# tjqansthd/GDN-Pytorch

Measured on AMD Instinct MI355X. Metric: training images/sec at 128x416 batch=20, higher is better.
Workload: dtype f32; 1 GPU; DtoD training step (fwd + losses + bwd + fused Adam), batch 20 per GPU, 128x416, fp32, BASELINE configs[1]; global_batch=20, parallelism=dp1, launch=eager, x3=True

## Files before the change

### gdn-pytorch_amd/csrc/conv_wino.hip

```cpp
#include "common.h"
#include "wino_gemm.h"
#include "up2x.h"
#include "gemm_x3.h"

namespace {

struct WinoGeom {
    int B, H, W, C, N;
    int Ho, Wo;
    int pad_off;
    int reflect;
    int tiles_y, tiles_x, M;
    int cq_shift, nq_shift;
    int x3;
    int flip;
    int T, bins;
};

__global__ __launch_bounds__(256) void wino_input_kernel(const float* __restrict__ x, int ldx, float* __restrict__ V, WinoGeom g,
                                                         const float* __restrict__ in_scale, const float* __restrict__ in_shift,
                                                         int in_relu, int up2x) {
    int t, c;
    if (!wino_decode(g.M, g.cq_shift, t, c)) return;
    const float is = in_scale ? in_scale[c] : 1.f, it = in_scale ? in_shift[c] : 0.f;
// ... 718 lines not shown
    WinoGeom f;
    if (!wino_geom(g, f)) return GDN_ERR_UNSUPPORTED;
    if (!dy || (!dx && !dw) || (dx && !w && !state) || (dw && !state)) return GDN_ERR_BAD_ARG;
    if (bnb_y && (!dx || !bnb_co || !bnb_partial)) return GDN_ERR_BAD_ARG;
    if (bnb_y && f.reflect) return GDN_ERR_UNSUPPORTED;
    if (dx && f.reflect && ((ldx % 4) || (addsrc && (ld_add % 4)))) return GDN_ERR_UNSUPPORTED;
    if (dx_up2x < 0 || dx_up2x > 2 || (dx_up2x && ((g->H & 1) || (g->W & 1)))) return GDN_ERR_BAD_ARG;
    if (dx && dx_up2x && !f.reflect) return GDN_ERR_UNSUPPORTED;
    if (!workspace || workspace_bytes < gdn_winoconv_bwd_workspace_bytes(g)) return GDN_ERR_WORKSPACE;
    hipStream_t st = (hipStream_t)stream;
    char* p = (char*)workspace;
    const size_t Md = f.reflect ? (size_t)f.B * cdiv(f.H + 2, 2) * cdiv(f.W + 2, 2) : (size_t)f.M;
    const size_t vd = al256((size_t)f.bins * Md * f.N * 4);
    float* Vd = (float*)p; p += (vd > m_bytes(f) ? vd : m_bytes(f));
    float* U = (float*)p; p += u_bytes(f);
    float* Eo = (float*)p;
    if (f.T == 4) {
        if (dw) {
            hipLaunchKernelGGL(wino4_dy_kernel, dim3(cdiv(f.M, 4) << f.nq_shift), dim3(256), 0, st, dy, ldy, Vd, f);
            const int ns = tn_splits(f);
            launch_gemm_x3_tn((const float*)Vd, (const float*)state, Eo, f.bins, f.M, f.N, f.C, ns, st);
            hipLaunchKernelGGL(wino4_wgrad_output_kernel, dim3(cdiv(f.N * f.C, 256)), dim3(256), 0, st, (const float*)Eo, dw, f.N, f.C, ns, f.flip ? 1 : 0);
        }
        if (dx) {
            WinoGeom fd = f;
            fd.C = f.N; fd.N = f.C; fd.cq_shift = f.nq_shift; fd.nq_shift = f.cq_shift;
            hipLaunchKernelGGL(wino4_input_kernel, dim3(cdiv(fd.M, 4) << fd.cq_shift), dim3(256), 0, st, dy, ldy, Vd, fd,
                               (const float*)nullptr, (const float*)nullptr, 0, 0);
            const float* Ud = U;
            if (state) Ud = (const float*)((const char*)state + v_bytes(f));
            else hipLaunchKernelGGL(wino4_weights_x3_kernel, dim3(cdiv(f.N * f.C / 8, 256)), dim3(256), 0, st, w, (unsigned char*)U, f.N, f.C, 1 | f.flip,
                                    (unsigned char*)nullptr, 0);
            launch_gemm_x3_nt((const float*)Vd, Ud, Eo, f.bins, fd.M, f.C, f.N, st);
            hipLaunchKernelGGL(wino4_output_kernel, dim3(cdiv(fd.M, 4) << fd.nq_shift), dim3(256), 0, st, (const float*)Eo, dx, ldx,
                               addsrc, ld_add, bnb_y ? bnb_partial : (float*)nullptr, (const float*)nullptr, (const float*)nullptr, 0,
                               fd, f.C, fd.nq_shift, bnb_y, ld_bnb, bnb_co, bnb_relu);
        }
        return gdn_launch_status();
    }
    if (dw) {
        hipLaunchKernelGGL(wino_dy_kernel, dim3(cdiv(f.M, 4) << f.nq_shift), dim3(256), 0, st, dy, ldy, Vd, f);
        const int ns = tn_splits(f);
        if (tn_x3(f)) launch_gemm_x3_tn((const float*)Vd, (const float*)state, Eo, WINO_BINS, f.M, f.N, f.C, ns, st);
        else launch_wino_gemm_tn((const float*)Vd, (const float*)state, Eo, f.M, f.N, f.C, ns, st);
        hipLaunchKernelGGL(wino_wgrad_output_kernel, dim3(cdiv(f.N * f.C, 256)), dim3(256), 0, st, (const float*)Eo, dw, f.N, f.C, ns, f.flip ? 1 : 0);
    }
    if (dx) {
        WinoGeom fd = f;
        fd.C = f.N; fd.N = f.C; fd.cq_shift = f.nq_shift; fd.nq_shift = f.cq_shift; fd.reflect = 0;
        float* out = dx;
        int ld_out = ldx;
        if (f.reflect) {
            fd.Ho = f.H + 2; fd.Wo = f.W + 2; fd.pad_off = 2;
            fd.tiles_y = cdiv(fd.Ho, 2); fd.tiles_x = cdiv(fd.Wo, 2); fd.M = f.B * fd.tiles_y * fd.tiles_x;
            out = Eo + (size_t)WINO_BINS * fd.M * f.C;
            ld_out = f.C;
        }
        hipLaunchKernelGGL(wino_input_kernel, dim3(cdiv(fd.M, 4) << fd.cq_shift), dim3(256), 0, st, dy, ldy, Vd, fd,
                           (const float*)nullptr, (const float*)nullptr, 0, 0);
        const float* Ud = U;
        const bool x3d = f.x3 && gemm_x3_ok(f.M, f.C, f.N);
        if (state) Ud = (const float*)((const char*)state + v_bytes(f));
        else if (x3d) hipLaunchKernelGGL(wino_weights_x3_kernel, dim3(cdiv(f.N * f.C / 8, 256)), dim3(256), 0, st, w, (unsigned char*)U, f.N, f.C, 1 | f.flip,
                                         (unsigned char*)nullptr, 0);
        else hipLaunchKernelGGL(wino_weights_kernel, dim3(cdiv(f.N * f.C, 256)), dim3(256), 0, st, w, U, f.N, f.C, 1 | f.flip, (float*)nullptr);
        if (x3d) launch_gemm_x3_nt((const float*)Vd, Ud, Eo, WINO_BINS, fd.M, f.C, f.N, st);
        else launch_wino_gemm((const float*)Vd, Ud, Eo, fd.M, f.C, f.N, st);
        hipLaunchKernelGGL(wino_output_kernel, dim3(cdiv(fd.M, 4) << fd.nq_shift), dim3(256), 0, st, (const float*)Eo, out, ld_out,
                           f.reflect ? (const float*)nullptr : addsrc, ld_add, bnb_y ? bnb_partial : (float*)nullptr,
                           (const float*)nullptr, (const float*)nullptr, 0, fd, f.C, fd.nq_shift, bnb_y, ld_bnb, bnb_co, bnb_relu);
        if (f.reflect && dx_up2x) {
            const int64_t nb = cdiv64((int64_t)f.B * (f.H / 2) * (f.W / 2) * (f.C / 4), 256);
            hipLaunchKernelGGL(reflect_fold_up2x_kernel, dim3((unsigned)(nb < 65536 * 8 ? nb : 65536 * 8)), dim3(256), 0, st,
                               (const void*)out, (void*)dx, ldx, (const void*)addsrc, ld_add, f.B, f.H, f.W, f.C, 1, dx_up2x - 1, 0);
        } else if (f.reflect) {
            const int64_t nb = cdiv64((int64_t)f.B * f.H * f.W * (f.C / 4), 256);
            hipLaunchKernelGGL(wino_reflect_fold_kernel, dim3((unsigned)(nb < 65536 * 8 ? nb : 65536 * 8)), dim3(256), 0, st,
                               (const float*)out, dx, ldx, addsrc, ld_add, f.B, f.H, f.W, f.C);
        }
    }
    return gdn_launch_status();
}

extern "C" int gdn_winoconv_gemm(const gdn_conv_geom* g, const float* V, const float* U, float* Mo, void* stream) {
    (void)hipGetLastError();
    WinoGeom f;
    if (!wino_geom(g, f)) return GDN_ERR_UNSUPPORTED;
    if (!V || !U || !Mo) return GDN_ERR_BAD_ARG;
    launch_wino_gemm(V, U, Mo, f.B * cdiv(f.H, 2) * cdiv(f.W, 2), f.N, f.C, (hipStream_t)stream);
    return gdn_launch_status();
}
```

### gdn-pytorch_amd/gdn_amd/_lib.py

```python
import ctypes
import os
import pathlib
from ctypes import POINTER, Structure, c_char_p, c_float, c_int32, c_int64, c_size_t, c_uint64, c_void_p

_PKG = pathlib.Path(__file__).resolve().parent
LIB_PATH = pathlib.Path(os.environ.get("GDN_HIP_LIB", _PKG.parent / "lib" / "libgdn_hip.so"))


class GdnError(RuntimeError):
    pass


class ConvGeom(Structure):
    _fields_ = [("B", c_int32), ("H", c_int32), ("W", c_int32), ("Cin", c_int32), ("Cout", c_int32),
                ("k", c_int32), ("stride", c_int32), ("pad", c_int32), ("pad_mode", c_int32),
                ("transposed", c_int32), ("hints", c_int32)]


_PG = POINTER(ConvGeom)
_P = c_void_p
_i32, _i64, _f, _sz = c_int32, c_int64, c_float, c_size_t

_SIGS = {
    "gdn_version": (c_int32, []),
    "gdn_hints_supported": (c_int32, []),
    "gdn_strerror": (c_char_p, [c_int32]),
    "gdn_device_info": (c_int32, [c_char_p, c_int32]),
    "gdn_conv_out_dims": (c_int32, [_PG, POINTER(c_int32), POINTER(c_int32)]),
    "gdn_conv_stats_slots": (_i64, [_PG, _i32]),
    "gdn_conv_fwd_workspace_bytes": (_sz, [_PG, _i32]),
    "gdn_conv_fwd": (c_int32, [_PG, _P, _i32, _P, _i32, _i32, _P, _P, _i32, _P, _i32, _P, _P, _P, _i32, _i32, _P, _sz, _P]),
    "gdn_conv_dgrad_workspace_bytes": (_sz, [_PG, _i32]),
    "gdn_conv_dgrad": (c_int32, [_PG, _P, _i32, _P, _P, _i32, _P, _i32, _P, _i32, _P, _i32, _P, _i32, _P, _sz, _i32, _P]),
    "gdn_conv_dgrad_bnb_slots": (_i64, [_PG, _i32]),
    "gdn_conv_wgrad_workspace_bytes": (_sz, [_PG, _i32]),
    "gdn_conv_wgrad": (c_int32, [_PG, _P, _i32, _i32, _P, _i32, _P, _i32, _i32, _P, _sz, _i32, _P]),
    "gdn_conv_wgrad_bf16_workspace_bytes": (_sz, [_PG, _i32, _i32]),
    "gdn_conv_wgrad_bf16": (c_int32, [_PG, _P, _i32, _i32, _P, _i32, _P, _i32, _i32, _P, _sz, _i32, _P]),
    "gdn_fftconv_fwd_workspace_bytes": (_sz, [_PG]),
    "gdn_fftconv_spectrum_bytes": (_sz, [_PG]),
    "gdn_fftconv_stats_slots": (_i64, [_PG]),
    "gdn_fftconv_fwd": (c_int32, [_PG, _P, _i32, _P, _P, _i32, _P, _i32, _P, _P, _P, _i32, _P, _P, _i32, _i32, _P, _P, _sz, _P]),
    "gdn_fftconv_bwd_workspace_bytes": (_sz, [_PG]),
    "gdn_fftconv_bwd": (c_int32, [_PG, _P, _i32, _P, _P, _P, _i32, _P, _i32, _P, _P, _i32, _P, _P, _i32, _P, _i32, _P, _i32, _P,
                                  _i32, _i32, _P, _sz, _P]),
    "gdn_fftconv_bnb_slots": (_i64, [_PG]),
    "gdn_fftconv_cgemm_workspace_bytes": (_sz, [_PG]),
    "gdn_fftconv_cgemm": (c_int32, [_PG, _i32, _P, _sz, _P]),
    "gdn_fftconv_cgemm_shape": (c_int32, [_PG, _P, _P, _P]),
    "gdn_winoconv_fwd_workspace_bytes": (_sz, [_PG]),
    "gdn_winoconv_state_bytes": (_sz, [_PG]),
    "gdn_winoconv_stats_slots": (_i64, [_PG]),
    "gdn_winoconv_fwd": (c_int32, [_PG, _P, _i32, _P, _P, _i32, _P, _i32, _P, _P, _P, _i32, _P, _P, _i32, _i32, _P, _P, _sz, _P]),
    "gdn_winoconv_bwd_workspace_bytes": (_sz, [_PG]),
    "gdn_winoconv_bnb_slots": (_i64, [_PG]),
    "gdn_winoconv_gemm": (c_int32, [_PG, _P, _P, _P, _P]),
    "gdn_winoconv_bwd": (c_int32, [_PG, _P, _i32, _P, _P, _P, _i32, _P, _i32, _P, _P, _i32, _P, _i32, _P, _i32, _P, _sz, _P]),
    "gdn_wino2conv_fwd_workspace_bytes": (_sz, [_PG]),
    "gdn_wino2conv_state_bytes": (_sz, [_PG]),
    "gdn_wino2conv_stats_slots": (_i64, [_PG]),
    "gdn_wino2conv_fwd": (c_int32, [_PG, _P, _i32, _P, _P, _i32, _P, _i32, _P, _P, _P, _i32, _P, _P, _sz, _P]),
    "gdn_wino2conv_bwd_workspace_bytes": (_sz, [_PG]),
    "gdn_wino2conv_bwd": (c_int32, [_PG, _P, _i32, _P, _P, _i32, _P, _P, _i32, _P, _i32, _P, _P, _sz, _P]),
    "gdn_conv_c1_stats_slots": (_i64, [_i32, _i32, _i32]),
    "gdn_conv_c1_fwd": (c_int32, [_P, _i32, _i32, _i32, _i32, _i32, _i32, _i32, _i32, _i32, _P, _P, _i32, _P, _i32, _P, _P, _P, _i32,
                                  _i32, _P]),
    "gdn_conv_c1_wgrad_workspace_bytes": (_sz, []),
    "gdn_conv_c1_wgrad": (c_int32, [_P, _P, _i32, _i32, _i32, _i32, _i32, _i32, _i32, _i32, _i32, _i32, _P, _P, _sz, _P]),
    "gdn_gemm_x3_packed_bytes": (_sz, [_i32, _i32, _i32]),
    "gdn_gemm_x3_pack": (c_int32, [_P, _P, _i32, _i32, _i32, _P]),
    "gdn_gemm_x3_nt": (c_int32, [_P, _P, _P, _i32, _i32, _i32, _i32, _P]),
    "gdn_gemm_x3_tn": (c_int32, [_P, _P, _P, _i32, _i32, _i32, _i32, _i32, _P]),
    "gdn_gemm_x3_tn_splits": (_i64, [_i32, _i32, _i32, _i32]),
    "gdn_transpose_taps": (c_int32, [_P, _P, _i32, _i32, _i32, _i32, _P]),
    "gdn_cast": (c_int32, [_P, _P, _i64, _i32, _P]),
    "gdn_weight_to_tapmajor": (c_int32, [_P, _P, _i32, _i32, _i32, _i32, _P]),
    "gdn_weight_from_tapmajor": (c_int32, [_P, _P, _i32, _i32, _i32, _i32, _P]),
    "gdn_bn_finalize_train": (c_int32, [_P, _i64, _i32, _i64, _P, _P, _P, _P, _f, _f, _P, _P, _P, _P, _P, _P]),
    "gdn_bn_eval_coeffs": (c_int32, [_P, _P, _P, _P, _f, _i32, _P, _P, _P]),
    "gdn_bn_apply": (c_int32, [_P, _i32, _P, _P, _P, _i32, _P, _i32, _i64, _i32, _i32, _i32, _P]),
    "gdn_bn_bwd_workspace_bytes": (_sz, [_i64, _i32]),
    "gdn_bn_bwd": (c_int32, [_P, _i32, _P, _i32, _P, _P, _P, _P, _P, _P, _i32, _P, _P, _i64, _i32, _i32, _P, _i64, _P, _sz, _i32, _P]),
    "gdn_bn_bwd_coeffs": (c_int32, [_P, _i32, _P, _i32, _P, _P, _P, _P, _P, _P, _P, _i64, _i32, _i32, _P, _i64, _P, _sz, _i32, _P]),
    "gdn_bn_eval_bwd": (c_int32, [_P, _i32, _P, _i32, _P, _P, _P, _i32, _i64, _i32, _i32, _i32, _P]),
    "gdn_bn_apply_up2x": (c_int32, [_P, _P, _P, _P, _P, _P, _i32, _i32, _i32, _i32, _i32, _i32, _i32, _P]),
    "gdn_upsample2x_fwd": (c_int32, [_P, _P, _i32, _i32, _i32, _i32, _i32, _i32, _P]),
    "gdn_upsample2x_bwd": (c_int32, [_P, _P, _i32, _i32, _i32, _i32, _i32, _i32, _P]),
    "gdn_nchw_to_nhwc": (c_int32, [_P, _P, _i32, _i32, _i32, _i32, _i32, _P]),
    "gdn_nhwc_to_nchw": (c_int32, [_P, _P, _i32, _i32, _i32, _i32, _i32, _P]),
    "gdn_add": (c_int32, [_P, _P, _P, _i64, _i32, _P]),
    "gdn_add_pitched": (c_int32, [_P, _i32, _P, _i32, _P, _i32, _i64, _i32, _i32, _P]),
    "gdn_scale_dev": (c_int32, [_P, _P, _P, _i64, _P]),
    "gdn_tanh_bwd": (c_int32, [_P, _P, _P, _i64, _P]),
    "gdn_fill": (c_int32, [_P, _f, _i64, _P]),
    "gdn_loss_workspace_bytes": (_sz, [_i64]),
    "gdn_absdiff_max": (c_int32, [_P, _P, _i64, _P, _P]),
    "gdn_berhu_masked": (c_int32, [_P, _P, _P, _i32, _i32, _i32, _i32, POINTER(c_int32), _P, _P, _P, _P, _sz, _P]),
    "gdn_sobel_l1": (c_int32, [_P, _P, _i32, _i32, _i32, _f, _P, _P, _P, _P, _P, _sz, _P]),
    "gdn_smoothness": (c_int32, [_P, _P, _i32, _i32, _i32, _i32, _P, _P, _P, _P, _P, _P, _sz, _P]),
    "gdn_mse": (c_int32, [_P, _P, _i64, _f, _i32, _P, _P, _sz, _i32, _P]),
    "gdn_kitti_augment_workspace_bytes": (_sz, [_i32]),
    "gdn_kitti_augment": (c_int32, [_P, _i32, _i32, _i32, _i32, _i32, _P, _i32, _P, _P, _sz, _P]),
    "gdn_kitti_augment_resident": (c_int32, [_P, _i32, _P, _i32, _P, _i32, _i32, _i32, _P, _i32, _i32, _P, _P, _P, _P]),
    "gdn_gather_samples": (c_int32, [_P, _i32, _P, _i32, _i64, _i32, _P, _P]),
    "gdn_mse_grad": (c_int32, [_P, _P, _i64, _f, _P, _P, _i32, _P]),
    "gdn_depth_metrics_workspace_bytes": (_sz, [_i32, _i32, _i32]),
    "gdn_depth_metrics": (c_int32, [_P, _P, _P, _i32, _i32, _i32, _i32, _P, _P, _sz, _P]),
    "gdn_depth_metrics_nyu_workspace_bytes": (_sz, [_i32, _i32, _i32]),
    "gdn_depth_metrics_nyu": (c_int32, [_P, _P, _i32, _i32, _i32, _i32, _P, _P, _sz, _P]),
    "gdn_depth_metrics_make3d_workspace_bytes": (_sz, [_i32, _i32, _i32]),
    "gdn_depth_metrics_make3d": (c_int32, [_P, _P, _P, _i32, _i32, _i32, _P, _P, _sz, _P]),
    "gdn_crop_normalize": (c_int32, [_P, _i32, _i32, _i32, _i32, _i32, _i32, _i32, _i32, _i32, _P, _P]),
    "gdn_bytescale_u8": (c_int32, [_P, _i32, _i32, _i32, _i32, _P, _P]),
    "gdn_nyu_augment_workspace_bytes": (_sz, [_i32, _i32, _i32, _i32]),
    "gdn_nyu_augment": (c_int32, [_P, _P, _i32, _i32, _i32, _i32, _P, _i32, _i32, _P, _P, _P, _sz, _P]),
    "gdn_pil_resize_workspace_bytes": (_sz, [_i32, _i32, _i32, _i32]),
    "gdn_pil_resize_bilinear": (c_int32, [_P, _i32, _i32, _i32, _i32, _i32, _i32, _i32, _i32, _i32, _i32, _i32, _i32, _i32,
                                          _P, _P, _sz, _P]),
    "gdn_spline_rotate3_workspace_bytes": (_sz, [_i32, _i32, _i32, _i32]),
    "gdn_spline_rotate3": (c_int32, [_P, _i32, _i32, _i32, _i32, _P, _P, _i32, _P, _P, _sz, _P]),
    "gdn_adam_step": (c_int32, [_P, _P, _P, _P, _i64, _f, _f, _f, _f, _f, _i32, _f, _P]),
    "gdn_adam_step_dev": (c_int32, [_P, _P, _P, _P, _i64, _P, _P, _P]),
    "gdn_clock_probe_arm": (c_int32, [_P, _P]),
    "gdn_clock_probe_watch": (c_int32, [_P, c_uint64, _P]),
    "gdn_clock_probe_stop": (c_int32, [_P, _P]),
}
_STATUS_FUNCS = {n for n, (r, _) in _SIGS.items() if r is c_int32} - {"gdn_version", "gdn_device_info", "gdn_hints_supported"}

EXPORTS = tuple(_SIGS)
ABI_VERSION = 223


class _Lib:
    def __init__(self):
        self._dll = None

    def _load(self):
        if self._dll is not None:
            return self._dll
        if not LIB_PATH.exists():
# ... 38 lines not shown
```

### gdn-pytorch_amd/gdn_amd/ops.py

```python
import ctypes
import math
import os

import numpy as np
import torch

from ._lib import ConvGeom, GdnError, lib

ACT_NONE, ACT_TANH, ACT_RELU = 0, 1, 2
BN_EPS, BN_MOMENTUM = 1e-5, 0.1


def stream():
    return torch.cuda.current_stream().cuda_stream


def _p(t):
    return None if t is None else t.data_ptr()


def _is_bf16(t):
    return 1 if t is not None and t.dtype == torch.bfloat16 else 0


# ... 359 lines not shown
                         device=dy.device) if need_dx else None
        ws = workspace(nb, dy.device, "fft")
        yy, yco, ykk, yrelu = dyb if dyb is not None else (None, None, None, False)

        def call(phases, st):
            lib.gdn_fftconv_bwd(ref, _p(dy), _ld(dy), _p(w_tap), _p(xf), _p(dx),
                                0 if dx is None else _ld(dx), _p(addsrc), 0 if addsrc is None else _ld(addsrc),
                                _p(dw_tap), _p(yy), 0 if yy is None else _ld(yy), _p(yco), _p(ykk), 1 if yrelu else 0,
                                _p(by), 0 if by is None else _ld(by), _p(bco), 1 if brelu else 0, _p(bpart),
                                int(up2x), phases, _p(ws), nb, st)
        if dw_tap is not None and need_dx:
            main = torch.cuda.current_stream(dy.device)
            side = side_stream(dy.device)
            call(1, main.cuda_stream)
            side.wait_stream(main)
            call(2, side.cuda_stream)
            call(4, main.cuda_stream)
            main.wait_stream(side)
        else:
            call(0, stream())
        return dx

    def fft_cgemm_only(self, B, H, W, which, ws=None, train=False, st=None):
        _, ref, _, _ = self.geom(B, H, W, hints=HINT_TRAIN if train else 0)
        nb = int(lib.gdn_fftconv_cgemm_workspace_bytes(ref))
        if nb == 0:
            raise GdnError("fftconv: unsupported layer k=%d stride=%d" % (self.k, self.stride))
        if ws is None:
            ws = torch.empty(nb // 4, dtype=torch.float32, device="cuda").normal_()
        lib.gdn_fftconv_cgemm(ref, int(which), _p(ws), nb, stream() if st is None else st)
        bins, M, npnt = ctypes.c_int32(), ctypes.c_int32(), ctypes.c_int32()
        lib.gdn_fftconv_cgemm_shape(ref, ctypes.byref(bins), ctypes.byref(M), ctypes.byref(npnt))
        return ws, bins.value, M.value, npnt.value

    def wino_ok(self, B, H, W, backward=False):
        _, ref, _, _ = self.geom(B, H, W)
        if backward:
            return int(lib.gdn_winoconv_bwd_workspace_bytes(ref)) > 0
        return int(lib.gdn_winoconv_state_bytes(ref)) > 0

    def wino_fwd(self, x, w_tap, stats=False, addsrc=None, state=False, affine=None, act=ACT_NONE, in_affine=None,
                 in_relu=False, up2x=0):
        _chk(x, "x"); _chk(w_tap, "w")
        B, H, W, C1 = x.shape
        if up2x:
            H, W = 2 * H, 2 * W
        _, ref, Ho, Wo = self.geom(B, H, W)
        nb = int(lib.gdn_winoconv_fwd_workspace_bytes(ref))
        if nb == 0 or C1 != self.cin:
            raise GdnError("winoconv: unsupported layer k=%d stride=%d Cin=%d Cout=%d" % (self.k, self.stride, C1, self.cout))
        y = torch.empty((B, Ho, Wo, self.cout), dtype=torch.float32, device=x.device)
        st = torch.empty((int(lib.gdn_winoconv_stats_slots(ref)), 2, self.cout), dtype=torch.float32,
                         device=x.device) if stats else None
        sv = torch.empty(int(lib.gdn_winoconv_state_bytes(ref)), dtype=torch.uint8, device=x.device) if state else None
        if sv is not None:
            sv._gdn_x3 = _x3
            sv._gdn_f4 = _f4
        ws = workspace(nb, x.device, "fft")
        lib.gdn_winoconv_fwd(ref, _p(x), _ld(x), _p(w_tap), _p(y), _ld(y), _p(addsrc), 0 if addsrc is None else _ld(addsrc),
                             _p(st), _p(affine[0]) if affine else None, _p(affine[1]) if affine else None, int(act),
                             _p(in_affine[0]) if in_affine else None, _p(in_affine[1]) if in_affine else None,
                             1 if in_relu else 0, int(up2x), _p(sv), _p(ws), nb, stream())
        res = (y,) + ((st,) if stats else ()) + ((sv,) if state else ())
        return res if len(res) > 1 else y

    def wino_gemm_only(self, V, U, Mo, B, H, W):
        _, ref, _, _ = self.geom(B, H, W)
        lib.gdn_winoconv_gemm(ref, _p(V), _p(U), _p(Mo), stream())

    def wino_bwd(self, dy, w_tap, in_hw, state=None, dw_tap=None, need_dx=True, addsrc=None, bnb=None, up2x=0):
        _chk(dy, "dy")
        B = dy.shape[0]
        H, W = in_hw
        _, ref, Ho, Wo = self.geom(B, H, W, x3=_state_x3(state), f4=_state_f4(state))
        nb = int(lib.gdn_winoconv_bwd_workspace_bytes(ref))
        if nb == 0:
            raise GdnError("winoconv: unsupported layer k=%d stride=%d" % (self.k, self.stride))
        if tuple(dy.shape[1:]) != (Ho, Wo, self.cout):
            raise GdnError("wino_bwd: dy shape %s does not match layer output" % (tuple(dy.shape),))
        if bnb is not None and not need_dx:
            raise GdnError("wino_bwd: bnb needs the data gradient (need_dx)")
        dx = torch.empty((B, H // 2, W // 2, self.cin) if up2x else (B, H, W, self.cin), dtype=torch.float32,
                         device=dy.device) if need_dx else None
        ws = workspace(nb, dy.device, "fft")
        by, bco, brelu, bpart = bnb if bnb is not None else (None, None, False, None)
        lib.gdn_winoconv_bwd(ref, _p(dy), _ld(dy), _p(w_tap), _p(state), _p(dx), 0 if dx is None else _ld(dx), _p(addsrc),
                             0 if addsrc is None else _ld(addsrc), _p(dw_tap), _p(by), 0 if by is None else _ld(by), _p(bco),
                             1 if brelu else 0, _p(bpart), int(up2x), _p(ws), nb, stream())
        return dx

    def wino2_ok(self, B, H, W):
        _, ref, _, _ = self.geom(B, H, W)
        return int(lib.gdn_wino2conv_fwd_workspace_bytes(ref)) > 0

    def wino2_fwd(self, x, w_tap, stats=False, addsrc=None, state=False, affine=None, act=ACT_NONE):
        _chk(x, "x"); _chk(w_tap, "w")
        B, H, W, C1 = x.shape
        _, ref, Ho, Wo = self.geom(B, H, W)
        nb = int(lib.gdn_wino2conv_fwd_workspace_bytes(ref))
        if nb == 0 or C1 != self.cin:
            raise GdnError("wino2conv: unsupported layer k=%d stride=%d Cin=%d Cout=%d" % (self.k, self.stride, C1, self.cout))
        y = torch.empty((B, Ho, Wo, self.cout), dtype=torch.float32, device=x.device)
        st = torch.empty((int(lib.gdn_wino2conv_stats_slots(ref)), 2, self.cout), dtype=torch.float32,
                         device=x.device) if stats else None
        sv = None
        if state:
            sb = int(lib.gdn_wino2conv_state_bytes(ref))
            sv = torch.empty(sb, dtype=torch.uint8, device=x.device) if sb else x
        ws = workspace(nb, x.device, "fft")
        lib.gdn_wino2conv_fwd(ref, _p(x), _ld(x), _p(w_tap), _p(y), _ld(y), _p(addsrc), 0 if addsrc is None else _ld(addsrc),
                              _p(st), _p(affine[0]) if affine else None, _p(affine[1]) if affine else None, int(act),
                              _p(sv) if (sv is not None and sv is not x) else None, _p(ws), nb, stream())
        res = (y,) + ((st,) if stats else ()) + ((sv,) if state else ())
        return res if len(res) > 1 else y

    def wino2_bwd(self, dy, w_tap, in_hw, state=None, dw_tap=None, need_dx=True, addsrc=None, bnb=None):
        _chk(dy, "dy")
        B = dy.shape[0]
        H, W = in_hw
        _, ref, Ho, Wo = self.geom(B, H, W)
        nb = int(lib.gdn_wino2conv_bwd_workspace_bytes(ref))
        if nb == 0:
            raise GdnError("wino2conv: unsupported layer k=%d stride=%d" % (self.k, self.stride))
        if tuple(dy.shape[1:]) != (Ho, Wo, self.cout):
            raise GdnError("wino2_bwd: dy shape %s does not match layer output" % (tuple(dy.shape),))
        dx = torch.empty((B, H, W, self.cin), dtype=torch.float32, device=dy.device) if need_dx else None
        ws = workspace(nb, dy.device, "fft")
        xin = state if self.transposed else None
        sv = None if self.transposed else state
        lib.gdn_wino2conv_bwd(ref, _p(dy), _ld(dy), _p(w_tap), _p(xin), 0 if xin is None else _ld(xin), _p(sv), _p(dx),
                              0 if dx is None else _ld(dx), _p(addsrc), 0 if addsrc is None else _ld(addsrc), _p(dw_tap),
                              _p(ws), nb, stream())
        return dx

    def wgrad(self, x, dy, dw_tap, ci_off=0, cfg=0):
        _chk(x, "x", bf16_ok=True)
        _chk(dy, "dy", bf16_ok=True)
        _chk(dw_tap, "dw")
        B, H, W, Cx = x.shape
        _, ref, _, _ = self.geom(B, H, W)
        if x.dtype == torch.bfloat16 and dy.dtype == torch.bfloat16:
            nb = int(lib.gdn_conv_wgrad_bf16_workspace_bytes(ref, Cx, cfg))
            if nb == 0:
                raise GdnError("bf16 wgrad: unsupported geometry k=%d stride=%d Cx=%d Cout=%d" % (self.k, self.stride, Cx, self.cout))
            ws = workspace(nb, x.device, "wgrad")
            lib.gdn_conv_wgrad_bf16(ref, _p(x), _ld(x), Cx, _p(dy), _ld(dy), _p(dw_tap), self.cin, ci_off, _p(ws), nb, cfg,
                                    stream())
            return
        nb = int(lib.gdn_conv_wgrad_workspace_bytes(ref, Cx))
        if nb == 0:
            raise GdnError("wgrad: unsupported geometry k=%d stride=%d Cx=%d" % (self.k, self.stride, Cx))
        ws = workspace(nb, x.device, "wgrad")
        lib.gdn_conv_wgrad(ref, _p(x), _ld(x), Cx, _p(dy), _ld(dy), _p(dw_tap), self.cin, ci_off, _p(ws), nb,
                           _mask(x, dy), stream())


def c1_ok(x1, n, k, stride, pad, rgb=False):
    return (x1.dtype == torch.float32 and x1.dim() == 4 and (x1.shape[3] == 1 or (rgb and x1.shape[3] == 3)) and x1.is_contiguous()
            and n == 64 and k == 9 and stride == 1 and pad == 4)


def conv_c1_fwd(x1, w81, reflect=False, flip=False, stats=False, addsrc=None, affine=None, act=ACT_NONE, out_dtype=torch.float32):
    _chk(x1, "x1"); _chk(w81, "w")
    if x1.dtype != torch.float32 or w81.dtype != torch.float32:
        raise GdnError("conv_c1_fwd: the image and the weights are fp32")
    B, H, W, cin = x1.shape
    if cin not in (1, 3) or w81.numel() != 81 * 64 * cin or not w81.is_contiguous() or not x1.is_contiguous():
        raise GdnError("conv_c1_fwd: dense [B,H,W,1|3] image and 81 x 64 x Cin contiguous weights expected")
# ... 520 lines not shown
```

### include/gdn_hip.h

```cpp
#ifndef GDN_HIP_H
#define GDN_HIP_H

#include <stddef.h>
#include <stdint.h>

#ifdef __cplusplus
extern "C" {
#endif

typedef enum {
    GDN_OK = 0,
    GDN_ERR_BAD_ARG = -1,
    GDN_ERR_UNSUPPORTED = -2,
    GDN_ERR_WORKSPACE = -3,
    GDN_ERR_LAUNCH = -4
} gdn_status;

int gdn_version(void);
int gdn_hints_supported(void);
const char* gdn_strerror(int status);
int gdn_device_info(char* name, int name_len);

typedef struct {
    int32_t B, H, W;
    int32_t Cin, Cout;
    int32_t k, stride, pad;
    int32_t pad_mode;
    int32_t transposed;
    int32_t hints;
} gdn_conv_geom;

enum { GDN_HINT_TRAIN = 1, GDN_HINT_NO_X3 = 2, GDN_HINT_NO_WINO_F4 = 4, GDN_HINT_FFT_NP32 = 8, GDN_HINT_FFT_NP40 = 16,
       GDN_HINT_FLIP_TAPS = 32 };
#define GDN_HINT_PLAN_BATCH(n) (((n) & 0xff) << 8)
#define GDN_HINT_PLAN_CUS(n) ((((n) / 8) & 0xff) << 16)

enum { GDN_ACT_NONE = 0, GDN_ACT_TANH = 1, GDN_ACT_RELU = 2 };

enum { GDN_CFG_KC64 = 0x200, GDN_CFG_NO_SPLITK = 0x800, GDN_CFG_BF16 = 0x10000 };

int gdn_conv_out_dims(const gdn_conv_geom* g, int32_t* Ho, int32_t* Wo);

int64_t gdn_conv_stats_slots(const gdn_conv_geom* g, int32_t tile_cfg);

size_t gdn_conv_fwd_workspace_bytes(const gdn_conv_geom* g, int32_t tile_cfg);
int gdn_conv_fwd(const gdn_conv_geom* g,
                 const void* x, int32_t ldx, const void* x2, int32_t ldx2, int32_t C1,
                 const void* w, void* y, int32_t ldy,
                 const void* addsrc, int32_t ld_add,
                 float* stats, const float* ep_scale, const float* ep_shift, int32_t act, int32_t tile_cfg,
                 void* workspace, size_t workspace_bytes, void* stream);

size_t gdn_conv_dgrad_workspace_bytes(const gdn_conv_geom* g, int32_t tile_cfg);
int64_t gdn_conv_dgrad_bnb_slots(const gdn_conv_geom* g, int32_t tile_cfg);
int gdn_conv_dgrad(const gdn_conv_geom* g, const void* dy, int32_t ldy,
                   const void* wt, void* dx, int32_t ldx,
                   const void* addsrc, int32_t ld_add,
                   const void* bnb_y, int32_t ld_bnb, const float* bnb_co, int32_t bnb_relu, float* bnb_partial,
                   int32_t dx_up2x, void* workspace, size_t workspace_bytes, int32_t tile_cfg, void* stream);

size_t gdn_conv_wgrad_workspace_bytes(const gdn_conv_geom* g, int32_t Cx);
int gdn_conv_wgrad(const gdn_conv_geom* g, const void* x, int32_t ldx, int32_t Cx,
                   const void* dy, int32_t ldy,
                   float* dw, int32_t ld_dw, int32_t ci_off,
                   void* workspace, size_t workspace_bytes, int32_t dtypes, void* stream);

size_t gdn_fftconv_fwd_workspace_bytes(const gdn_conv_geom* g);
size_t gdn_fftconv_spectrum_bytes(const gdn_conv_geom* g);
int64_t gdn_fftconv_stats_slots(const gdn_conv_geom* g);
int gdn_fftconv_fwd(const gdn_conv_geom* g, const float* x, int32_t ldx, const float* w,
                    float* y, int32_t ldy, const float* addsrc, int32_t ld_add, float* stats,
                    const float* ep_scale, const float* ep_shift, int32_t act,
                    const float* in_scale, const float* in_shift, int32_t in_relu, int32_t in_up2x,
                    void* xf_out, void* workspace, size_t workspace_bytes, void* stream);
enum { GDN_FFT_BWD_TRANSFORM = 1, GDN_FFT_BWD_DW = 2, GDN_FFT_BWD_DX = 4, GDN_FFT_BWD_ALL = 7 };
size_t gdn_fftconv_bwd_workspace_bytes(const gdn_conv_geom* g);
int gdn_fftconv_bwd(const gdn_conv_geom* g, const float* dy, int32_t ldy, const float* w,
                    const void* xf, float* dx, int32_t ldx, const float* addsrc, int32_t ld_add,
                    float* dw, const float* dyb_y, int32_t ld_dyb, const float* dyb_co,
                    const float* dyb_kk, int32_t dyb_relu,
                    const float* bnb_y, int32_t ld_bnb, const float* bnb_co, int32_t bnb_relu, float* bnb_partial,
                    int32_t dx_up2x, int32_t phases,
                    void* workspace, size_t workspace_bytes, void* stream);
int64_t gdn_fftconv_bnb_slots(const gdn_conv_geom* g);
size_t gdn_fftconv_cgemm_workspace_bytes(const gdn_conv_geom* g);
int gdn_fftconv_cgemm(const gdn_conv_geom* g, int32_t which, void* workspace, size_t workspace_bytes, void* stream);
int gdn_fftconv_cgemm_shape(const gdn_conv_geom* g, int32_t* bins, int32_t* M, int32_t* np);

size_t gdn_winoconv_fwd_workspace_bytes(const gdn_conv_geom* g);
size_t gdn_winoconv_state_bytes(const gdn_conv_geom* g);
int64_t gdn_winoconv_stats_slots(const gdn_conv_geom* g);
int gdn_winoconv_fwd(const gdn_conv_geom* g, const float* x, int32_t ldx, const float* w,
                     float* y, int32_t ldy, const float* addsrc, int32_t ld_add, float* stats,
                     const float* ep_scale, const float* ep_shift, int32_t act,
                     const float* in_scale, const float* in_shift, int32_t in_relu, int32_t in_up2x,
                     void* state_out, void* workspace, size_t workspace_bytes, void* stream);
size_t gdn_winoconv_bwd_workspace_bytes(const gdn_conv_geom* g);
int64_t gdn_winoconv_bnb_slots(const gdn_conv_geom* g);
int gdn_winoconv_gemm(const gdn_conv_geom* g, const float* V, const float* U, float* Mo, void* stream);
int gdn_winoconv_bwd(const gdn_conv_geom* g, const float* dy, int32_t ldy, const float* w,
                     const void* state, float* dx, int32_t ldx, const float* addsrc, int32_t ld_add,
                     float* dw, const float* bnb_y, int32_t ld_bnb, const float* bnb_co, int32_t bnb_relu,
                     float* bnb_partial, int32_t dx_up2x, void* workspace, size_t workspace_bytes, void* stream);

size_t gdn_wino2conv_fwd_workspace_bytes(const gdn_conv_geom* g);
size_t gdn_wino2conv_state_bytes(const gdn_conv_geom* g);
int64_t gdn_wino2conv_stats_slots(const gdn_conv_geom* g);
int gdn_wino2conv_fwd(const gdn_conv_geom* g, const float* x, int32_t ldx, const float* w,
                      float* y, int32_t ldy, const float* addsrc, int32_t ld_add, float* stats,
                      const float* ep_scale, const float* ep_shift, int32_t act,
                      void* state_out, void* workspace, size_t workspace_bytes, void* stream);
size_t gdn_wino2conv_bwd_workspace_bytes(const gdn_conv_geom* g);
int gdn_wino2conv_bwd(const gdn_conv_geom* g, const float* dy, int32_t ldy, const float* w,
                      const float* x, int32_t ldx_in, const void* state,
                      float* dx, int32_t ldx, const float* addsrc, int32_t ld_add, float* dw,
                      void* workspace, size_t workspace_bytes, void* stream);

int64_t gdn_conv_c1_stats_slots(int32_t B, int32_t H, int32_t W);
int gdn_conv_c1_fwd(const float* x1, int32_t Cin, int32_t B, int32_t H, int32_t W, int32_t N, int32_t k, int32_t pad, int32_t reflect,
                    int32_t flip, const float* w, void* y, int32_t ldy, const void* addsrc, int32_t ld_add,
                    float* stats, const float* ep_scale, const float* ep_shift, int32_t act, int32_t dtypes, void* stream);
size_t gdn_conv_c1_wgrad_workspace_bytes(void);
int gdn_conv_c1_wgrad(const float* x1, const void* gw, int32_t ldg, int32_t gw_bf16, int32_t B, int32_t H, int32_t W, int32_t N,
                      int32_t k, int32_t pad, int32_t reflect, int32_t flip, float* dw,
                      void* workspace, size_t workspace_bytes, void* stream);

size_t gdn_gemm_x3_packed_bytes(int32_t bins, int32_t rows, int32_t K);
int gdn_gemm_x3_pack(const float* src, void* dst, int32_t bins, int32_t rows, int32_t K, void* stream);
int gdn_gemm_x3_nt(const float* A, const void* Bp, float* C, int32_t bins, int32_t M, int32_t N, int32_t K, void* stream);
int gdn_gemm_x3_tn(const float* A, const float* B, float* P, int32_t bins, int32_t T, int32_t NI, int32_t NJ, int32_t nsplit,
                   void* stream);
int64_t gdn_gemm_x3_tn_splits(int32_t bins, int32_t T, int32_t NI, int32_t NJ);

size_t gdn_conv_wgrad_bf16_workspace_bytes(const gdn_conv_geom* g, int32_t Cx, int32_t cfg);
int gdn_conv_wgrad_bf16(const gdn_conv_geom* g, const void* x, int32_t ldx, int32_t Cx,
                        const void* dy, int32_t ldy,
                        float* dw, int32_t ld_dw, int32_t ci_off,
                        void* workspace, size_t workspace_bytes, int32_t cfg, void* stream);


int gdn_transpose_taps(const void* w, void* wt, int32_t ntaps, int32_t R, int32_t C, int32_t dtypes, void* stream);
int gdn_cast(const void* src, void* dst, int64_t n, int32_t dtypes, void* stream);
int gdn_weight_to_tapmajor(const float* w_torch, float* w_tap, int32_t Cout, int32_t Cin, int32_t ntaps,
                           int32_t a_is_cout, void* stream);
int gdn_weight_from_tapmajor(const float* w_tap, float* w_torch, int32_t Cout, int32_t Cin, int32_t ntaps,
                             int32_t a_is_cout, void* stream);

int gdn_bn_finalize_train(const float* stats, int64_t slots, int32_t C, int64_t count,
                          const float* gamma, const float* beta,
                          float* running_mean, float* running_var, float momentum, float eps,
                          float* scale, float* shift, float* mean, float* invstd,
                          int64_t* num_batches_tracked, void* stream);
int gdn_bn_eval_coeffs(const float* gamma, const float* beta, const float* running_mean,
                       const float* running_var, float eps, int32_t C,
                       float* scale, float* shift, void* stream);
int gdn_bn_apply(const void* y, int32_t ldy, const float* scale, const float* shift,
                 const void* residual, int32_t ld_res, void* out, int32_t ld_out,
                 int64_t npix, int32_t C, int32_t relu, int32_t dtypes, void* stream);
int gdn_bn_apply_up2x(const void* y, const float* scale, const float* shift, const void* residual, void* low, void* up,
                      int32_t B, int32_t H, int32_t W, int32_t C, int32_t relu, int32_t align_corners, int32_t dtypes,
                      void* stream);
size_t gdn_bn_bwd_workspace_bytes(int64_t npix, int32_t C);
int gdn_bn_bwd(const void* dout, int32_t ld_dout, const void* y, int32_t ldy,
               const float* gamma, const float* scale, const float* shift,
               const float* mean, const float* invstd,
               void* dy, int32_t ld_dy, float* dgamma, float* dbeta,
               int64_t npix, int32_t C, int32_t relu,
               const float* ext_partial, int64_t ext_slots,
               void* workspace, size_t workspace_bytes, int32_t dtypes, void* stream);

int gdn_bn_bwd_coeffs(const void* dout, int32_t ld_dout, const void* y, int32_t ldy,
                      const float* scale, const float* shift, const float* mean, const float* invstd,
                      float* dgamma, float* dbeta, float* kk, int64_t npix, int32_t C, int32_t relu,
                      const float* ext_partial, int64_t ext_slots,
                      void* workspace, size_t workspace_bytes, int32_t dtypes, void* stream);

int gdn_bn_eval_bwd(const void* dout, int32_t ld_dout, const void* y, int32_t ldy,
                    const float* scale, const float* shift, void* dy, int32_t ld_dy,
                    int64_t npix, int32_t C, int32_t relu, int32_t dtypes, void* stream);

int gdn_upsample2x_fwd(const void* x, void* y, int32_t B, int32_t H, int32_t W, int32_t C,
                       int32_t align_corners, int32_t dtypes, void* stream);
int gdn_upsample2x_bwd(const void* dy, void* dx, int32_t B, int32_t H, int32_t W, int32_t C,
                       int32_t align_corners, int32_t dtypes, void* stream);

int gdn_nchw_to_nhwc(const void* x, void* y, int32_t B, int32_t C, int32_t H, int32_t W, int32_t dtypes, void* stream);
// ... 100 lines not shown
```

Measured before the change: 528.5 images/s.

## Overlap Winograd-4 weight-grad and data-grad GEMMs on separate streams

Adds a phased Winograd F(4) backward entry point that splits the input transforms, the weight-gradient GEMM and reduction, and the data-gradient GEMM and output transform into selectable phases. The Python wrapper runs the transforms on the main stream, then the wgrad phase on a side stream while dgrad runs on the main stream, and joins the two afterwards. The aim is to fill GPU idle time by running the two independent backward GEMMs at the same time. In exchange it needs a larger workspace holding both transformed buffers, adds stream synchronisation overhead, and skips the up2x and non-T=4 cases.

```diff
diff --git a/gdn-pytorch_amd/csrc/conv_wino.hip b/gdn-pytorch_amd/csrc/conv_wino.hip
--- a/gdn-pytorch_amd/csrc/conv_wino.hip
+++ b/gdn-pytorch_amd/csrc/conv_wino.hip
@@ -824,6 +824,63 @@
     return gdn_launch_status();
 }
 
+namespace {
+inline size_t pair_vd_bytes(const WinoGeom& f) { return al256((size_t)f.bins * f.M * f.N * 4); }
+inline size_t pair_p_bytes(const WinoGeom& f) { return (size_t)tn_splits_max(f) * al256((size_t)f.bins * f.N * f.C * 4); }
+inline size_t pair_eo_bytes(const WinoGeom& f) { return al256((size_t)f.bins * f.M * f.C * 4); }
+inline bool pair_geom(const gdn_conv_geom* g, WinoGeom& f) { return wino_geom(g, f) && f.T == 4; }
+}
+
+extern "C" size_t gdn_winoconv_bwd_pair_workspace_bytes(const gdn_conv_geom* g) {
+    WinoGeom f;
+    if (!pair_geom(g, f)) return 0;
+    return 2 * pair_vd_bytes(f) + pair_p_bytes(f) + pair_eo_bytes(f);
+}
+
+extern "C" int gdn_winoconv_bwd_pair(const gdn_conv_geom* g, const float* dy, int32_t ldy, const float* w, const void* state,
+                                     float* dx, int32_t ldx, const float* addsrc, int32_t ld_add, float* dw,
+                                     const float* bnb_y, int32_t ld_bnb, const float* bnb_co, int32_t bnb_relu,
+                                     float* bnb_partial, int32_t dx_up2x, int32_t phases, void* workspace, size_t workspace_bytes,
+                                     void* stream) {
+    (void)hipGetLastError();
+    (void)w;
+    WinoGeom f;
+    if (!pair_geom(g, f)) return GDN_ERR_UNSUPPORTED;
+    if (!dy || !dx || !dw || !state) return GDN_ERR_BAD_ARG;
+    if (bnb_y && (!bnb_co || !bnb_partial)) return GDN_ERR_BAD_ARG;
+    if (dx_up2x < 0 || dx_up2x > 2) return GDN_ERR_BAD_ARG;
+    if (dx_up2x) return GDN_ERR_UNSUPPORTED;
+    if (phases < 0 || phases > 7) return GDN_ERR_BAD_ARG;
+    if (!workspace || workspace_bytes < gdn_winoconv_bwd_pair_workspace_bytes(g)) return GDN_ERR_WORKSPACE;
+    if (!phases) phases = 7;
+    hipStream_t st = (hipStream_t)stream;
+    char* p = (char*)workspace;
+    float* Vd = (float*)p; p += pair_vd_bytes(f);
+    float* Dv = (float*)p; p += pair_vd_bytes(f);
+    float* P = (float*)p; p += pair_p_bytes(f);
+    float* Eo = (float*)p;
+    WinoGeom fd = f;
+    fd.C = f.N; fd.N = f.C; fd.cq_shift = f.nq_shift; fd.nq_shift = f.cq_shift;
+    if (phases & 1) {
+        hipLaunchKernelGGL(wino4_input_kernel, dim3(cdiv(fd.M, 4) << fd.cq_shift), dim3(256), 0, st, dy, ldy, Vd, fd,
+                           (const float*)nullptr, (const float*)nullptr, 0, 0);
+        hipLaunchKernelGGL(wino4_dy_kernel, dim3(cdiv(f.M, 4) << f.nq_shift), dim3(256), 0, st, dy, ldy, Dv, f);
+    }
+    if (phases & 2) {
+        const int ns = tn_splits(f);
+        launch_gemm_x3_tn((const float*)Dv, (const float*)state, P, f.bins, f.M, f.N, f.C, ns, st);
+        hipLaunchKernelGGL(wino4_wgrad_output_kernel, dim3(cdiv(f.N * f.C, 256)), dim3(256), 0, st, (const float*)P, dw, f.N, f.C, ns, f.flip ? 1 : 0);
+    }
+    if (phases & 4) {
+        const float* Ud = (const float*)((const char*)state + v_bytes(f));
+        launch_gemm_x3_nt((const float*)Vd, Ud, Eo, f.bins, fd.M, f.C, f.N, st);
+        hipLaunchKernelGGL(wino4_output_kernel, dim3(cdiv(fd.M, 4) << fd.nq_shift), dim3(256), 0, st, (const float*)Eo, dx, ldx,
+                           addsrc, ld_add, bnb_y ? bnb_partial : (float*)nullptr, (const float*)nullptr, (const float*)nullptr, 0,
+                           fd, f.C, fd.nq_shift, bnb_y, ld_bnb, bnb_co, bnb_relu);
+    }
+    return gdn_launch_status();
+}
+
 extern "C" int gdn_winoconv_gemm(const gdn_conv_geom* g, const float* V, const float* U, float* Mo, void* stream) {
     (void)hipGetLastError();
     WinoGeom f;
diff --git a/gdn-pytorch_amd/gdn_amd/_lib.py b/gdn-pytorch_amd/gdn_amd/_lib.py
--- a/gdn-pytorch_amd/gdn_amd/_lib.py
+++ b/gdn-pytorch_amd/gdn_amd/_lib.py
@@ -56,6 +56,9 @@
     "gdn_winoconv_bnb_slots": (_i64, [_PG]),
     "gdn_winoconv_gemm": (c_int32, [_PG, _P, _P, _P, _P]),
     "gdn_winoconv_bwd": (c_int32, [_PG, _P, _i32, _P, _P, _P, _i32, _P, _i32, _P, _P, _i32, _P, _i32, _P, _i32, _P, _sz, _P]),
+    "gdn_winoconv_bwd_pair_workspace_bytes": (_sz, [_PG]),
+    "gdn_winoconv_bwd_pair": (c_int32, [_PG, _P, _i32, _P, _P, _P, _i32, _P, _i32, _P, _P, _i32, _P, _i32, _P, _i32, _i32, _P, _sz,
+                                        _P]),
     "gdn_wino2conv_fwd_workspace_bytes": (_sz, [_PG]),
     "gdn_wino2conv_state_bytes": (_sz, [_PG]),
     "gdn_wino2conv_stats_slots": (_i64, [_PG]),
diff --git a/gdn-pytorch_amd/gdn_amd/ops.py b/gdn-pytorch_amd/gdn_amd/ops.py
--- a/gdn-pytorch_amd/gdn_amd/ops.py
+++ b/gdn-pytorch_amd/gdn_amd/ops.py
@@ -465,8 +465,24 @@
             raise GdnError("wino_bwd: bnb needs the data gradient (need_dx)")
         dx = torch.empty((B, H // 2, W // 2, self.cin) if up2x else (B, H, W, self.cin), dtype=torch.float32,
                          device=dy.device) if need_dx else None
+        by, bco, brelu, bpart = bnb if bnb is not None else (None, None, False, None)
+        npair = int(lib.gdn_winoconv_bwd_pair_workspace_bytes(ref)) if dw_tap is not None and need_dx and not up2x else 0
+        if npair and state is not None:
+            ws = workspace(npair, dy.device, "fft")
+
+            def call(phases, st):
+                lib.gdn_winoconv_bwd_pair(ref, _p(dy), _ld(dy), _p(w_tap), _p(state), _p(dx), _ld(dx), _p(addsrc),
+                                          0 if addsrc is None else _ld(addsrc), _p(dw_tap), _p(by), 0 if by is None else _ld(by),
+                                          _p(bco), 1 if brelu else 0, _p(bpart), 0, phases, _p(ws), npair, st)
+            main = torch.cuda.current_stream(dy.device)
+            side = side_stream(dy.device)
+            call(1, main.cuda_stream)
+            side.wait_stream(main)
+            call(2, side.cuda_stream)
+            call(4, main.cuda_stream)
+            main.wait_stream(side)
+            return dx
         ws = workspace(nb, dy.device, "fft")
-        by, bco, brelu, bpart = bnb if bnb is not None else (None, None, False, None)
         lib.gdn_winoconv_bwd(ref, _p(dy), _ld(dy), _p(w_tap), _p(state), _p(dx), 0 if dx is None else _ld(dx), _p(addsrc),
                              0 if addsrc is None else _ld(addsrc), _p(dw_tap), _p(by), 0 if by is None else _ld(by), _p(bco),
                              1 if brelu else 0, _p(bpart), int(up2x), _p(ws), nb, stream())
diff --git a/include/gdn_hip.h b/include/gdn_hip.h
--- a/include/gdn_hip.h
+++ b/include/gdn_hip.h
@@ -102,6 +102,12 @@
                      const void* state, float* dx, int32_t ldx, const float* addsrc, int32_t ld_add,
                      float* dw, const float* bnb_y, int32_t ld_bnb, const float* bnb_co, int32_t bnb_relu,
                      float* bnb_partial, int32_t dx_up2x, void* workspace, size_t workspace_bytes, void* stream);
+size_t gdn_winoconv_bwd_pair_workspace_bytes(const gdn_conv_geom* g);
+int gdn_winoconv_bwd_pair(const gdn_conv_geom* g, const float* dy, int32_t ldy, const float* w,
+                          const void* state, float* dx, int32_t ldx, const float* addsrc, int32_t ld_add,
+                          float* dw, const float* bnb_y, int32_t ld_bnb, const float* bnb_co, int32_t bnb_relu,
+                          float* bnb_partial, int32_t dx_up2x, int32_t phases, void* workspace, size_t workspace_bytes,
+                          void* stream);
 
 size_t gdn_wino2conv_fwd_workspace_bytes(const gdn_conv_geom* g);
 size_t gdn_wino2conv_state_bytes(const gdn_conv_geom* g);
```

New measurement: 538.8 images/s, median of 6. 1.9% higher.
